# tridivb/attention_based_tbn

Measured on AMD Instinct MI355X. Metric: clips/sec (3-seg RGB+Flow+Audio TBN fwd+bwd), higher is better.
Workload: dtype f32; 1 GPU; BASELINE config 4: RGB+Flow+Audio async, attention off, 3 segments, 224x224 frames + 1.279 s (256x256) spectrogram, train step fwd+loss+bwd+clip+SGD; batch_per_gpu=32, global_batch=32, segments=3, parallelism=single, launch_plans=committed (bench_plans.json)

## Files before the change

### attention_based_tbn_amd/build.py

```python
import os
import subprocess
import sys
from concurrent.futures import ThreadPoolExecutor

HERE = os.path.dirname(os.path.abspath(__file__))
CSRC = os.path.join(HERE, "csrc")
LIB = os.path.join(HERE, "libtbn_hip.so")
SOURCES = ["api.hip", "conv_igemm.hip", "conv_bf16x.hip", "bn.hip", "bn_multi.hip", "bn_res.hip", "pool.hip", "heads.hip", "stft.hip", "engine.hip", "train_ops.hip", "frames.hip", "jpeg.hip", "jpeg_entropy.hip", "audio_load.hip", "inflate.hip", "deflate.hip", "audio_stem.hip", "vgg_ops.hip"]
FLAGS = ["--offload-arch=gfx950", "-O3", "-fPIC", "-std=c++17", "-Wall", "-Wno-unused-function",
         "-mllvm", "-amdgpu-mfma-vgpr-form",
         "-I" + os.path.join(os.path.dirname(HERE), "include")]
if os.environ.get("TBN_DIAG") == "1":
    FLAGS.append("-DTBN_DIAG=1")
if os.environ.get("TBN_EXTRA_FLAGS"):
    FLAGS += os.environ["TBN_EXTRA_FLAGS"].split()
if os.environ.get("TBN_ABLATE") == "1":
    FLAGS.append("-DTBN_ABLATE=1")
if os.environ.get("TBN_EXPERIMENT") == "1":
    FLAGS.append("-DTBN_EXPERIMENT=1")


def _hipcc():
    for c in (os.environ.get("HIPCC"), "/opt/rocm/bin/hipcc", "hipcc"):
        if c and (os.path.isabs(c) and os.path.exists(c) or not os.path.isabs(c)):
            return c
    raise RuntimeError("hipcc not found")


def _stale(target, deps):
    if not os.path.exists(target):
        return True
    t = os.path.getmtime(target)
    return any(os.path.getmtime(d) > t for d in deps)


VARIANT = os.environ.get("TBN_BUILD_VARIANT")
if not VARIANT and any(os.environ.get(k) == "1" for k in ("TBN_EXPERIMENT", "TBN_DIAG", "TBN_ABLATE")):
    VARIANT = "exp" if os.environ.get("TBN_EXPERIMENT") == "1" else ("diag" if os.environ.get("TBN_DIAG") == "1" else "ablate")
OBJDIR = CSRC
if VARIANT:
    _ab = os.path.join(os.path.dirname(HERE), "scripts", "ab")
    OBJDIR = os.path.join(_ab, "obj_" + VARIANT)
    LIB = os.path.join(_ab, "lib_" + VARIANT + ".so")
    os.makedirs(OBJDIR, exist_ok=True)
STAMP = os.path.join(OBJDIR, ".build_flags")


def build(force=False, verbose=True):
    hipcc = _hipcc()
    flagset = " ".join(FLAGS)
    try:
        with open(STAMP) as f:
            if f.read() != flagset:
                force = True
    except OSError:
        force = force or any(os.path.exists(os.path.join(OBJDIR, s.replace(".hip", ".o"))) for s in SOURCES)
    headers = [os.path.join(CSRC, f) for f in os.listdir(CSRC) if f.endswith(".h")]
    headers.append(os.path.join(os.path.dirname(HERE), "include", "tbn_hip.h"))
    objs, jobs = [], []
    for s in SOURCES:
        src = os.path.join(CSRC, s)
        obj = os.path.join(OBJDIR, s.replace(".hip", ".o"))
        objs.append(obj)
        if force or _stale(obj, [src] + headers):
            jobs.append([hipcc] + FLAGS + ["-c", src, "-o", obj])

    def run(cmd):
        if verbose:
            print(" ".join(cmd), flush=True)
        r = subprocess.run(cmd, capture_output=True, text=True)
        if r.returncode != 0:
            raise RuntimeError("hipcc failed:\n" + r.stdout + r.stderr)
        if verbose and r.stderr.strip():
            print(r.stderr, file=sys.stderr)

    with ThreadPoolExecutor(max_workers=min(8, max(1, len(jobs)))) as ex:
        list(ex.map(run, jobs))
    with open(STAMP, "w") as f:
        f.write(flagset)
    if jobs or force or _stale(LIB, objs):
        run([hipcc, "--offload-arch=gfx950", "-shared", "-fPIC", "-o", LIB] + objs)
    return LIB


if __name__ == "__main__":
    print(build(force="--force" in sys.argv))
```

### attention_based_tbn_amd/csrc/bn.hip

```cpp
#include "tbn_common.h"
#include "tbn_kernels.h"
#include "tbn_bn_dev.h"
#include "tbn_pool_dev.h"

static inline int pick_chunk(int P, int rp) {
  int pch = cdiv(P, 512);
  if (pch < 64) pch = 64;
  return cdiv(pch, rp) * rp;
}

__global__ __launch_bounds__(256) void bn_stats_kernel(const float* __restrict__ y, int ld, int P, int C, int pch,
                                                       float* __restrict__ partial) {
  __shared__ float red[2 * 2048];
  const int G = C >> 2, RP = 256 / G;
  const int tid = threadIdx.x, cg = tid % G, rs = tid / G;
  const int p0 = blockIdx.x * pch, p1 = min(P, p0 + pch);
  float4 s1 = make_float4(0, 0, 0, 0), s2 = s1;
  if (rs < RP)
    for (int p = p0 + rs; p < p1; p += RP) {
      const float4 v = *reinterpret_cast<const float4*>(y + (size_t)p * ld + cg * 4);
      s1.x += v.x; s1.y += v.y; s1.z += v.z; s1.w += v.w;
      s2.x = fmaf(v.x, v.x, s2.x); s2.y = fmaf(v.y, v.y, s2.y); s2.z = fmaf(v.z, v.z, s2.z); s2.w = fmaf(v.w, v.w, s2.w);
    }
  if (rs < RP) {
// ... 22 lines not shown
              "bn_stats: P >= 1, C a multiple of 4 in 4..1024, pitch a multiple of 4 and at least C");
  const int rp = 256 / (C / 4), pch = pick_chunk(P, rp), parts = cdiv(P, pch);
  TBN_KLAUNCH(bn_stats_kernel, dim3(parts), dim3(256), 0, st, y, ld, P, C, pch, partial);
  TBN_CHECK_LAUNCH("bn_stats");
  if (nparts) *nparts = parts;
  return TBN_OK;
}

__global__ __launch_bounds__(256) void bn_finalize_kernel(const float* __restrict__ partial, int nparts, int P, int C,
                                                          const float* __restrict__ gamma,
                                                          const float* __restrict__ beta,
                                                          const float* __restrict__ conv_bias, float* running_mean,
                                                          float* running_var, float momentum, float eps,
                                                          float* save_mean, float* save_rstd, float* scale,
                                                          float* shift) {
  __shared__ double red[64 * 32];
  const int tid = threadIdx.x;
  const int c = blockIdx.x * TBN_FIN_CH + tid;
  double s1, s2;
  tbn_sum_partials<TBN_FIN_CH>(partial, C, nparts, blockIdx.x * TBN_FIN_CH, C, red, &s1, &s2);
  if (tid < TBN_FIN_CH && c < C) {
    const double mean = s1 / P;
    double var = s2 / P - mean * mean;
    if (var < 0.0) var = 0.0;
    const float rstd = (float)(1.0 / sqrt(var + (double)eps));
    const float sc = gamma[c] * rstd;
    save_mean[c] = (float)mean;
    save_rstd[c] = rstd;
    scale[c] = sc;
    shift[c] = fmaf(-(float)mean, sc, beta[c]);
    if (running_mean != nullptr) {
      const double unb = P > 1 ? var * ((double)P / (double)(P - 1)) : var;
      const float mean_b = (float)mean + (conv_bias != nullptr ? conv_bias[c] : 0.f);
      running_mean[c] = (1.f - momentum) * running_mean[c] + momentum * mean_b;
      running_var[c] = (1.f - momentum) * running_var[c] + momentum * (float)unb;
    }
  }
}

int tbn_launch_bn_finalize(const float* partial, int nparts, int P, int C, const float* gamma, const float* beta,
                           const float* conv_bias, float* running_mean, float* running_var, float momentum, float eps,
                           float* save_mean, float* save_rstd, float* scale, float* shift, hipStream_t st) {
  TBN_KLAUNCH(bn_finalize_kernel, dim3(cdiv(C, TBN_FIN_CH)), dim3(256), 0, st, partial, nparts, P, C, gamma, beta,
                     conv_bias, running_mean, running_var, momentum, eps, save_mean, save_rstd, scale, shift);
  TBN_CHECK_LAUNCH("bn_finalize");
  return TBN_OK;
}

struct Seg3 {
  Seg s[3];
  int n;
};
struct CSeg3 {
  CSeg s[3];
  int n;
};

__global__ __launch_bounds__(256) void bn_apply_kernel(const float* __restrict__ y, int P, int C,
                                                       const float* __restrict__ scale,
                                                       const float* __restrict__ shift, Seg3 segs, FastDiv divg) {
  const int G = C >> 2;
  const uint32_t total = (uint32_t)P * G;
  for (uint32_t i = blockIdx.x * 256u + threadIdx.x; i < total; i += gridDim.x * 256u) {
    const int p = (int)fdiv(i, divg), c = (int)(i - (uint32_t)p * (uint32_t)G) * 4;
    const float4 v = *reinterpret_cast<const float4*>(y + (size_t)p * C + c);
    const float4 sc = *reinterpret_cast<const float4*>(scale + c);
    const float4 sh = *reinterpret_cast<const float4*>(shift + c);
    float4 z;
// ... 481 lines not shown
```

### attention_based_tbn_amd/csrc/bn_multi.hip

```cpp
#include <cstdlib>
#include <cstring>
#include "tbn_common.h"
#include "tbn_kernels.h"
#include "tbn_bn_dev.h"
#include "tbn_rider_dev.h"

namespace {

__device__ __forceinline__ int find_layer(const int* blk0, int n, int b) {
  int l = 0;
  while (l + 1 < n && b >= blk0[l + 1]) ++l;
  return l;
}

#ifndef TBN_DIAG
#define TBN_DIAG 0
#endif
inline bool diag_skip_fin(int bit) {
#if TBN_DIAG
  static const int mask = getenv("TBN_DIAG_SKIP") ? atoi(getenv("TBN_DIAG_SKIP")) : 0;
  return (mask & bit) != 0;
#else
  (void)bit;
  return false;
#endif
}

inline int ew_grid(size_t items) {
  size_t g = (items + 255) / 256;
  return (int)(g > 4096 ? 4096 : (g < 1 ? 1 : g));
}

}

__global__ __launch_bounds__(256) void bn_finalize_multi_kernel(BnFwdBatch b) {
  __shared__ double red[64 * 32];
  const int li = find_layer(b.fin_blk0, b.n, blockIdx.x);
  const BnFwdLayer& L = b.l[li];
  const int blk = blockIdx.x - b.fin_blk0[li];
  const int C = L.C, P = L.P;
  const int tid = threadIdx.x;
  const int c = blk * TBN_FIN_CH + tid;
  double s1, s2;
  tbn_sum_partials<TBN_FIN_CH>(L.partial, L.pld, L.nparts, blk * TBN_FIN_CH, C, red, &s1, &s2);
  if (tid < TBN_FIN_CH && c < C) {
    const double mean = s1 / P;
    double var = s2 / P - mean * mean;
    if (var < 0.0) var = 0.0;
    const float rstd = (float)(1.0 / sqrt(var + (double)b.eps));
    const float sc = L.gamma[c] * rstd;
    L.save_mean[c] = (float)mean;
    L.save_rstd[c] = rstd;
    L.scale[c] = sc;
    L.shift[c] = fmaf(-(float)mean, sc, L.beta[c]);
    if (L.running_mean != nullptr) {
      const double unb = P > 1 ? var * ((double)P / (double)(P - 1)) : var;
      const float mean_b = (float)mean + (L.conv_bias != nullptr ? L.conv_bias[c] : 0.f);
      L.running_mean[c] = (1.f - b.momentum) * L.running_mean[c] + b.momentum * mean_b;
      L.running_var[c] = (1.f - b.momentum) * L.running_var[c] + b.momentum * (float)unb;
    }
  }
}

__global__ __launch_bounds__(256) void bn_apply_multi_kernel(BnFwdBatch b) {
  const int li = find_layer(b.app_blk0, b.n, blockIdx.x);
  const BnFwdLayer& L = b.l[li];
  const int blk = blockIdx.x - b.app_blk0[li];
  const int p0 = blk * L.app_rows, p1 = min(L.P, p0 + L.app_rows);
  if (L.nseg == 1 && L.seg[0].col_begin == 0) {
    tbn_bn_apply_rows(L.y, L.y_ld, L.seg[0].ptr, L.seg[0].ld, L.scale, L.shift, L.C, p0, p1);
    return;
  }
  const int G = L.C >> 2, RP = 256 / G;
  const int cg = threadIdx.x % G, rs = threadIdx.x / G;
  if (rs >= RP) return;
  const int c = cg * 4;
  const float4 sc = *reinterpret_cast<const float4*>(L.scale + c);
  const float4 sh = *reinterpret_cast<const float4*>(L.shift + c);
  int sg = 0;
  if (L.nseg > 1 && c >= L.seg[1].col_begin) sg = 1;
  if (L.nseg > 2 && c >= L.seg[2].col_begin) sg = 2;
  const float* yp = L.y + (size_t)(p0 + rs) * L.y_ld + c;
  float* zp = L.seg[sg].ptr + (size_t)(p0 + rs) * L.seg[sg].ld + (c - L.seg[sg].col_begin);
  const size_t ystep = (size_t)RP * L.y_ld, zstep = (size_t)RP * L.seg[sg].ld;
  int p = p0 + rs;
  for (; p + 3 * RP < p1; p += 4 * RP) {
    float4 v[4];
#pragma unroll
    for (int k = 0; k < 4; ++k) v[k] = *reinterpret_cast<const float4*>(yp + k * ystep);
#pragma unroll
    for (int k = 0; k < 4; ++k) {
      float4 z;
      z.x = fmaxf(fmaf(v[k].x, sc.x, sh.x), 0.f);
      z.y = fmaxf(fmaf(v[k].y, sc.y, sh.y), 0.f);
      z.z = fmaxf(fmaf(v[k].z, sc.z, sh.z), 0.f);
      z.w = fmaxf(fmaf(v[k].w, sc.w, sh.w), 0.f);
      *reinterpret_cast<float4*>(zp + k * zstep) = z;
    }
    yp += 4 * ystep;
    zp += 4 * zstep;
  }
  for (; p < p1; p += RP) {
    const float4 v = *reinterpret_cast<const float4*>(yp);
    float4 z;
    z.x = fmaxf(fmaf(v.x, sc.x, sh.x), 0.f);
    z.y = fmaxf(fmaf(v.y, sc.y, sh.y), 0.f);
    z.z = fmaxf(fmaf(v.z, sc.z, sh.z), 0.f);
    z.w = fmaxf(fmaf(v.w, sc.w, sh.w), 0.f);
    *reinterpret_cast<float4*>(zp) = z;
    yp += ystep;
    zp += zstep;
  }
}

static inline int apply_rows(int P, int C) {
  const int RP = 256 / (C / 4);
  int it = cdiv(P, RP * 2048);
  if (it < 4) it = 4;
  if (it > 16) it = 16;
  return RP * it;
}

int tbn_launch_bn_fwd_multi(BnFwdBatch& b, hipStream_t st) { return tbn_launch_bn_fwd_multi_defer(b, 0u, nullptr, st); }

int tbn_rider_place(RiderP* r, int gemm_blocks) {
  static const int front = tbn_env_int("TBN_RIDER_FRONT", 0, 0, 1);
  if (r == nullptr || r->nblk <= 0) return gemm_blocks;
  if (front) {
    r->span = (r->nblk + 7) / 8 * 8;
    r->first = 0;
    r->gemm0 = r->span;
  } else {
    r->span = r->nblk;
    r->first = gemm_blocks;
    r->gemm0 = 0;
  }
  return gemm_blocks + r->span;
}

int tbn_launch_bn_fwd_multi_defer(BnFwdBatch& b, unsigned defer_mask, RiderP* rider, hipStream_t st) {
  TBN_REQUIRE(b.n >= 1 && b.n <= TBN_BN_MAXL, "bn_fwd_multi: %d layers", b.n);
  TBN_REQUIRE(defer_mask == 0u || rider != nullptr, "bn_fwd_multi: deferred members need a rider descriptor");
  b.fin_blk0[0] = b.app_blk0[0] = 0;
  for (int i = 0; i < b.n; ++i) {
    BnFwdLayer& L = b.l[i];
    TBN_REQUIRE(L.P >= 1 && L.C >= 4 && L.C % 4 == 0 && L.C <= 1024 && L.y_ld % 4 == 0 && L.y_ld >= L.C && L.pld >= L.C &&
                L.pld % 4 == 0 && L.nparts >= 1 && L.nseg >= 1 && L.nseg <= 3, "bn_fwd_multi: bad P / C / pitch / nparts / nseg");
    for (int s = 0; s < L.nseg; ++s)
      TBN_REQUIRE(L.seg[s].ld % 4 == 0 && L.seg[s].col_begin % 4 == 0, "bn_fwd_multi: segment pitch/offset must be x4");
    b.fin_blk0[i + 1] = b.fin_blk0[i] + cdiv(L.C, TBN_FIN_CH);
    L.app_rows = apply_rows(L.P, L.C);
    b.app_blk0[i + 1] = b.app_blk0[i] + cdiv(L.P, L.app_rows);
  }
  if (!diag_skip_fin(16)) TBN_KLAUNCH(bn_finalize_multi_kernel, dim3(b.fin_blk0[b.n]), dim3(256), 0, st, b);
  TBN_CHECK_LAUNCH("bn_finalize_multi");
  if (defer_mask == 0u) {
    TBN_KLAUNCH(bn_apply_multi_kernel, dim3(b.app_blk0[b.n]), dim3(256), 0, st, b);
    TBN_CHECK_LAUNCH("bn_apply_multi");
    return TBN_OK;
  }
  static thread_local BnFwdBatch now;
  now.n = 0;
  now.momentum = b.momentum;
  now.eps = b.eps;
  now.app_blk0[0] = 0;
  memset(rider, 0, sizeof(*rider));
  rider->kind = 1;
  for (int i = 0; i < b.n; ++i) {
    const BnFwdLayer& L = b.l[i];
    const int blocks = b.app_blk0[i + 1] - b.app_blk0[i];
    if (defer_mask & (1u << i)) {
      TBN_REQUIRE(rider->n < TBN_RIDER_MAXL && L.nseg == 1 && L.seg[0].col_begin == 0, "bn_fwd_multi: rider holds at most %d single-segment layers", TBN_RIDER_MAXL);
      RiderLayer& R = rider->l[rider->n];
      R.y = L.y; R.y_ld = L.y_ld; R.out = L.seg[0].ptr; R.out_ld = L.seg[0].ld;
      R.scale = L.scale; R.shift = L.shift; R.P = L.P; R.C = L.C; R.rows = L.app_rows;
      rider->blk0[rider->n + 1] = rider->blk0[rider->n] + blocks;
      ++rider->n;
    } else {
      now.l[now.n] = L;
      now.app_blk0[now.n + 1] = now.app_blk0[now.n] + blocks;
      ++now.n;
    }
  }
  rider->nblk = rider->blk0[rider->n];
  if (now.n > 0) {
    TBN_KLAUNCH(bn_apply_multi_kernel, dim3(now.app_blk0[now.n]), dim3(256), 0, st, now);
    TBN_CHECK_LAUNCH("bn_apply_multi");
  }
  return TBN_OK;
}

__global__ __launch_bounds__(256) void bn_bwd_reduce_multi_kernel(BnBwdBatch b) {
  __shared__ float red[2 * 2048];
  const int li = find_layer(b.red_blk0, b.n, blockIdx.x);
  const BnBwdLayer& L = b.l[li];
  const int blk = blockIdx.x - b.red_blk0[li];
  const int C = L.C, P = L.P, pch = L.pch;
  const int G = C >> 2, RP = 256 / G;
  const int tid = threadIdx.x, cg = tid % G, rs = tid / G, c = cg * 4;
  const int p0 = blk * pch, p1 = min(P, p0 + pch);
  float4 s1 = make_float4(0, 0, 0, 0), s2 = s1;
  if (rs < RP) {
    int sg = 0;
    if (L.nseg > 1 && c >= L.dz[1].col_begin) sg = 1;
    if (L.nseg > 2 && c >= L.dz[2].col_begin) sg = 2;
    const float* dzp = L.dz[sg].ptr + (c - L.dz[sg].col_begin);
    const int dld = L.dz[sg].ld;
    const float4 sc = *reinterpret_cast<const float4*>(L.scale + c);
// ... 28 lines not shown
    L.partial[((size_t)blk * 2 + 0) * C + cc] = a;
    L.partial[((size_t)blk * 2 + 1) * C + cc] = s;
  }
}

__global__ __launch_bounds__(256) void bn_bwd_finalize_multi_kernel(BnBwdBatch b) {
  __shared__ double red[64 * 32];
  const int li = find_layer(b.fin_blk0, b.n, blockIdx.x);
  const BnBwdLayer& L = b.l[li];
  const int blk = blockIdx.x - b.fin_blk0[li];
  const int C = L.C, P = L.P;
  const int tid = threadIdx.x;
  const int c = blk * TBN_FIN_CH + tid;
  double s1, s2;
  tbn_sum_partials<TBN_FIN_CH>(L.partial, C, L.nparts, blk * TBN_FIN_CH, C, red, &s1, &s2);
  if (tid < TBN_FIN_CH && c < C) {
    const double sc = L.scale[c], rs = L.rstd[c], mu = L.mean[c];
    const double bb = -sc * rs * (s2 / P);
    L.coef[c] = (float)sc;
    L.coef[C + c] = (float)bb;
    L.coef[2 * C + c] = (float)(-sc * (s1 / P) - bb * mu);
    if (L.dgamma) L.dgamma[c] = (float)s2;
    if (L.dbeta) L.dbeta[c] = (float)s1;
    if (L.dbias) L.dbias[c] = 0.f;
  }
}

__global__ __launch_bounds__(256) void bn_bwd_apply_multi_kernel(BnBwdBatch b) {
  const int li = find_layer(b.app_blk0, b.n, blockIdx.x);
  const BnBwdLayer& L = b.l[li];
  const int blk = blockIdx.x - b.app_blk0[li];
  const int p0 = blk * L.app_rows, p1 = min(L.P, p0 + L.app_rows);
  if (L.nseg == 1 && L.dz[0].col_begin == 0) {
    tbn_bn_bwd_apply_rows(L.dz[0].ptr, L.dz[0].ld, L.y, L.y_ld, L.dy, L.scale, L.shift, L.coef, L.C, p0, p1);
    return;
  }
  const int C = L.C, G = C >> 2, RP = 256 / G;
  const int cg = threadIdx.x % G, rs = threadIdx.x / G;
  if (rs >= RP) return;
  const int c = cg * 4;
  int sg = 0;
  if (L.nseg > 1 && c >= L.dz[1].col_begin) sg = 1;
  if (L.nseg > 2 && c >= L.dz[2].col_begin) sg = 2;
  const float4 sc = *reinterpret_cast<const float4*>(L.scale + c);
  const float4 sh = *reinterpret_cast<const float4*>(L.shift + c);
  const float4 ca = *reinterpret_cast<const float4*>(L.coef + c);
  const float4 cb = *reinterpret_cast<const float4*>(L.coef + C + c);
  const float4 cc = *reinterpret_cast<const float4*>(L.coef + 2 * C + c);
  const float* dp = L.dz[sg].ptr + (size_t)(p0 + rs) * L.dz[sg].ld + (c - L.dz[sg].col_begin);
  const float* yp = L.y + (size_t)(p0 + rs) * L.y_ld + c;
  float* op = L.dy + (size_t)(p0 + rs) * L.y_ld + c;
  const size_t dstep = (size_t)RP * L.dz[sg].ld, ystep = (size_t)RP * L.y_ld;
  auto one = [&](const float4 d, const float4 v) {
    float4 o;
    o.x = fmaf(ca.x, fmaf(v.x, sc.x, sh.x) > 0.f ? d.x : 0.f, fmaf(cb.x, v.x, cc.x));
    o.y = fmaf(ca.y, fmaf(v.y, sc.y, sh.y) > 0.f ? d.y : 0.f, fmaf(cb.y, v.y, cc.y));
    o.z = fmaf(ca.z, fmaf(v.z, sc.z, sh.z) > 0.f ? d.z : 0.f, fmaf(cb.z, v.z, cc.z));
    o.w = fmaf(ca.w, fmaf(v.w, sc.w, sh.w) > 0.f ? d.w : 0.f, fmaf(cb.w, v.w, cc.w));
    return o;
  };
  int p = p0 + rs;
  for (; p + 3 * RP < p1; p += 4 * RP) {
    float4 d[4], v[4];
#pragma unroll
    for (int k = 0; k < 4; ++k) {
      d[k] = *reinterpret_cast<const float4*>(dp + k * dstep);
      v[k] = *reinterpret_cast<const float4*>(yp + k * ystep);
// ... 9 lines not shown
    dp += dstep;
    yp += ystep;
    op += ystep;
  }
}

int tbn_launch_bn_bwd_multi(BnBwdBatch& b, hipStream_t st) { return tbn_launch_bn_bwd_multi_defer(b, 0u, nullptr, st); }

int tbn_launch_bn_bwd_multi_defer(BnBwdBatch& b, unsigned defer_mask, RiderP* rider, hipStream_t st) {
  TBN_REQUIRE(b.n >= 1 && b.n <= TBN_BN_MAXL, "bn_bwd_multi: %d layers", b.n);
  TBN_REQUIRE(defer_mask == 0u || rider != nullptr, "bn_bwd_multi: deferred members need a rider descriptor");
  b.red_blk0[0] = b.fin_blk0[0] = b.app_blk0[0] = 0;
  for (int i = 0; i < b.n; ++i) {
    BnBwdLayer& L = b.l[i];
    TBN_REQUIRE(L.P >= 1 && L.C >= 4 && L.C % 4 == 0 && L.C <= 1024 && L.y_ld % 4 == 0 && L.y_ld >= L.C && L.ext_parts >= 0 &&
                L.nseg >= 1 && L.nseg <= 3, "bn_bwd_multi: bad P / C / pitch / ext_parts / nseg");
    for (int s = 0; s < L.nseg; ++s)
      TBN_REQUIRE(L.dz[s].ld % 4 == 0 && L.dz[s].col_begin % 4 == 0, "bn_bwd_multi: segment pitch/offset must be x4");
    {
      const int rp = 256 / (L.C / 4);
      int pch = cdiv(L.P, 512);
      if (pch < 64) pch = 64;
      L.pch = cdiv(pch, rp) * rp;
      L.nparts = cdiv(L.P, L.pch);
    }
    int red_blocks = L.nparts;
    if (L.ext_parts > 0) {
      L.nparts = L.ext_parts;
      red_blocks = 0;
    }
    b.red_blk0[i + 1] = b.red_blk0[i] + red_blocks;
    b.fin_blk0[i + 1] = b.fin_blk0[i] + cdiv(L.C, TBN_FIN_CH);
    L.app_rows = apply_rows(L.P, L.C);
    b.app_blk0[i + 1] = b.app_blk0[i] + cdiv(L.P, L.app_rows);
  }
  if (b.red_blk0[b.n] > 0) {
    TBN_KLAUNCH(bn_bwd_reduce_multi_kernel, dim3(b.red_blk0[b.n]), dim3(256), 0, st, b);
    TBN_CHECK_LAUNCH("bn_bwd_reduce_multi");
  }
  if (!diag_skip_fin(32)) TBN_KLAUNCH(bn_bwd_finalize_multi_kernel, dim3(b.fin_blk0[b.n]), dim3(256), 0, st, b);
  TBN_CHECK_LAUNCH("bn_bwd_finalize_multi");
  if (defer_mask == 0u) {
    TBN_KLAUNCH(bn_bwd_apply_multi_kernel, dim3(b.app_blk0[b.n]), dim3(256), 0, st, b);
    TBN_CHECK_LAUNCH("bn_bwd_apply_multi");
    return TBN_OK;
  }
  static thread_local BnBwdBatch now;
  now.n = 0;
  now.app_blk0[0] = 0;
  memset(rider, 0, sizeof(*rider));
  rider->kind = 2;
  for (int i = 0; i < b.n; ++i) {
    const BnBwdLayer& L = b.l[i];
    const int blocks = b.app_blk0[i + 1] - b.app_blk0[i];
    if (defer_mask & (1u << i)) {
      TBN_REQUIRE(rider->n < TBN_RIDER_MAXL && L.nseg == 1 && L.dz[0].col_begin == 0, "bn_bwd_multi: rider holds at most %d single-segment layers", TBN_RIDER_MAXL);
      RiderLayer& R = rider->l[rider->n];
      R.y = L.y; R.y_ld = L.y_ld; R.out = L.dy; R.out_ld = L.y_ld; R.dz = L.dz[0].ptr; R.dz_ld = L.dz[0].ld;
      R.scale = L.scale; R.shift = L.shift; R.coef = L.coef; R.P = L.P; R.C = L.C; R.rows = L.app_rows;
      rider->blk0[rider->n + 1] = rider->blk0[rider->n] + blocks;
      ++rider->n;
    } else {
      now.l[now.n] = L;
      now.app_blk0[now.n + 1] = now.app_blk0[now.n] + blocks;
      ++now.n;
    }
  }
  rider->nblk = rider->blk0[rider->n];
  if (now.n > 0) {
    TBN_KLAUNCH(bn_bwd_apply_multi_kernel, dim3(now.app_blk0[now.n]), dim3(256), 0, st, now);
    TBN_CHECK_LAUNCH("bn_bwd_apply_multi");
  }
  return TBN_OK;
}
```

### attention_based_tbn_amd/csrc/tbn_bn_dev.h

```cpp
#pragma once
#include "tbn_common.h"

#ifndef TBN_FIN_CH
#define TBN_FIN_CH 16
#endif

template <int CH>
__device__ __forceinline__ void tbn_sum_partials(const float* __restrict__ partial, int pld, int nparts, int c0, int C,
                                                 double* red, double* out_s1, double* out_s2) {
  constexpr int Q = CH / 4, S = 256 / Q, V = Q * 8, G = S / 8;
  static_assert(CH == 4 || CH == 8 || CH == 16, "finalize: 4, 8 or 16 channels per workgroup");
  const int tid = threadIdx.x, cq = tid % Q, slot = tid / Q;
  const int c = c0 + cq * 4;
  double a0 = 0, a1 = 0, a2 = 0, a3 = 0, b0 = 0, b1 = 0, b2 = 0, b3 = 0;
  if (c < C) {
    const float* p = partial + c;
    for (int i = slot; i < nparts; i += 4 * S) {
      float4 u[4], v[4];
#pragma unroll
      for (int k = 0; k < 4; ++k) {
        const int r = i + S * k;
        const bool ok = r < nparts;
        const size_t rr = (size_t)(ok ? r : i);
        u[k] = *reinterpret_cast<const float4*>(p + (rr * 2 + 0) * pld);
        v[k] = *reinterpret_cast<const float4*>(p + (rr * 2 + 1) * pld);
        if (!ok) u[k] = v[k] = make_float4(0.f, 0.f, 0.f, 0.f);
      }
#pragma unroll
      for (int k = 0; k < 4; ++k) {
        a0 += (double)u[k].x; a1 += (double)u[k].y; a2 += (double)u[k].z; a3 += (double)u[k].w;
        b0 += (double)v[k].x; b1 += (double)v[k].y; b2 += (double)v[k].z; b3 += (double)v[k].w;
      }
    }
  }
  double* r = red + slot * V + cq * 8;
  r[0] = a0; r[1] = a1; r[2] = a2; r[3] = a3;
  r[4] = b0; r[5] = b1; r[6] = b2; r[7] = b3;
  __syncthreads();
// ... 19 lines not shown
```

### attention_based_tbn_amd/csrc/tbn_kernels.h

```cpp
#pragma once
#include "tbn_common.h"
#include <hip/hip_ext.h>
#include <type_traits>

enum { CONV_EPI_PLAIN = 0, CONV_EPI_STATS = 1, CONV_EPI_EVAL = 2 };
enum {
  CONV_FLAG_ACCUM = 1,
  CONV_FLAG_RELU = 2,
  CONV_FLAG_HALO = 4,
  CONV_FLAG_DMA = 8,
  CONV_FLAG_SK4 = 16,
  CONV_FLAG_BF16X6 = 32,
  CONV_FLAG_BF16X3 = 64,
  CONV_FLAG_BF16X_PLANES = 128,
  CONV_FLAG_DESC_OUT2 = 256
};

#define TBN_CONV_MAXSEG 4
struct RedSeg {
  const float* y;
  float* partial;
  const float* stats;
  int y_ld, col_begin, C, c_off;
  unsigned y_bytes;
// ... 14 lines not shown
  int nred;
  int red_chan;
  int red_row0;
  int N, H, W;
  int OH, OW;
  int Cin;
  int Cout;
  int R, S, stride, pad, up;
  int M, K;
  int cp;
  int tiles_m, tiles_n;
  int mode, flags;
  double alg_flops;
  int stages;
  int halo;
  unsigned in_bytes, wt_bytes;
  unsigned seg_bytes[TBN_CONV_MAXSEG];
  int OHs, OWs;
  int out_sy, out_oy, out_sx, out_ox;
  int in_sy, in_sx;
  int Krow;
  int ntaps;
  int tap_dy[9], tap_dx[9];
  int tap_koff[9];
  int tap_off[9];
  int ty0, tny, tx0, tnx;
  FastDiv div_ohw, div_ow;
  FastDiv div_rl4;
  const float* fold_scale;
  const float* fold_shift;
};

#define TBN_RIDER_MAXL 3
struct RiderLayer {
  const float* y;
  const float* dz;
  float* out;
  const float* scale;
  const float* shift;
  const float* coef;
  int y_ld, dz_ld, out_ld, P, C, rows;
};
struct RiderP {
  int span;
  int first;
  int gemm0;
  int nblk;
  int kind;
  int n;
  int blk0[TBN_RIDER_MAXL + 1];
  RiderLayer l[TBN_RIDER_MAXL];
};
int tbn_rider_place(RiderP* r, int gemm_blocks);

struct WgradP {
  const float* dy;
  const float* x;
  float* out;
  int dy_ld, x_ld;
  int N, H, W, OH, OW;
  int Cin, Cout;
  int R, S, stride, pad;
  int taps;
  int M, K;
  int cp, rl;
  int tiles_co, tiles_ci;
  int rows_per_split;
  int mt, nt;
  FastDiv div_ohw, div_ow, div_rl4;
  unsigned mul_ow;
  unsigned r64;
  unsigned frame_bytes;
  unsigned fb_lo, fb_hi;
  unsigned row_step, col_step;
// ... 137 lines not shown
};
int tbn_launch_weight_flip_transpose_all(const float* w, float* wt, const FlipTab& tab, hipStream_t st);

int tbn_launch_bn_stats(const float* y, int ld, int P, int C, float* partial, int* nparts, hipStream_t st);
int tbn_bn_stats_parts(int P, int C);
int tbn_launch_bn_finalize(const float* partial, int nparts, int P, int C, const float* gamma, const float* beta,
                           const float* conv_bias, float* running_mean, float* running_var, float momentum, float eps,
                           float* save_mean, float* save_rstd, float* scale, float* shift, hipStream_t st);
int tbn_launch_bn_apply(const float* y, int P, int C, const float* scale, const float* shift, const Seg* segs,
                        int nseg, hipStream_t st);
int tbn_launch_bn_apply_maxpool(const float* y, int N, int H, int W, int C, const float* scale, const float* shift,
                                float* out, int out_ld, unsigned char* argmax, int OH, int OW, int stride, int pad,
                                hipStream_t st);
int tbn_launch_bn_bwd_reduce_pooled(const float* dpooled, int dpooled_ld, const unsigned char* argmax, int N, int H,
                                    int W, int OH, int OW, int stride, int pad, const float* y, int C,
                                    const float* scale, const float* shift, const float* mean, const float* rstd,
                                    float* partial, hipStream_t st);
int tbn_bn_bwd_pooled_parts(int N, int H, int W, int C, int stride, int pad);
int tbn_launch_bn_bwd_apply_pooled(const float* dpooled, int dpooled_ld, const unsigned char* argmax, int N, int H, int W,
                                   int OH, int OW, int stride, int pad, const float* y, int C, const float* scale,
                                   const float* shift, const float* coef, float* dy, hipStream_t st);
#define TBN_BN_MAXL 4
struct BnFwdLayer {
  const float* y;
  int y_ld;
  int P, C;
  const float* partial;
  int pld, nparts;
  const float *gamma, *beta, *conv_bias;
  float *running_mean, *running_var, *save_mean, *save_rstd, *scale, *shift;
  Seg seg[3];
  int nseg;
  int app_rows;
};
struct BnFwdBatch {
  int n;
  float momentum, eps;
  BnFwdLayer l[TBN_BN_MAXL];
  int fin_blk0[TBN_BN_MAXL + 1], app_blk0[TBN_BN_MAXL + 1];
};
struct BnBwdLayer {
  CSeg dz[3];
  int nseg;
  const float* y;
  float* dy;
  int y_ld;
  int P, C;
  const float *scale, *shift, *mean, *rstd;
  float* partial;
  int ext_parts;
  float* coef;
  float *dgamma, *dbeta, *dbias;
  int pch, nparts;
  int app_rows;
};
struct BnBwdBatch {
  int n;
  BnBwdLayer l[TBN_BN_MAXL];
  int red_blk0[TBN_BN_MAXL + 1], fin_blk0[TBN_BN_MAXL + 1], app_blk0[TBN_BN_MAXL + 1];
};
int tbn_launch_bn_fwd_multi(BnFwdBatch& b, hipStream_t st);
int tbn_launch_bn_bwd_multi(BnBwdBatch& b, hipStream_t st);
int tbn_launch_bn_fwd_multi_defer(BnFwdBatch& b, unsigned defer_mask, RiderP* rider, hipStream_t st);
int tbn_launch_bn_bwd_multi_defer(BnBwdBatch& b, unsigned defer_mask, RiderP* rider, hipStream_t st);
bool tbn_prof_enabled();
int tbn_launch_bn_fold(const float* gamma, const float* beta, const float* mean, const float* var, const float* bias,
                       float eps, float* scale, float* shift, int C, hipStream_t st);
int tbn_bn_bwd_parts(int P, int C);
int tbn_launch_bn_bwd_reduce(const CSeg* dz, int nseg, const float* y, int P, int C, const float* scale,
                             const float* shift, const float* mean, const float* rstd, float* partial, hipStream_t st);
int tbn_launch_bn_bwd_finalize(const float* partial, int nparts, int P, int C, const float* scale, const float* mean,
                               const float* rstd, float* coef, float* dgamma, float* dbeta, float* dbias,
                               hipStream_t st);
int tbn_launch_bn_bwd_apply(const CSeg* dz, int nseg, const float* y, int P, int C, const float* scale,
                            const float* shift, const float* coef, float* dy, hipStream_t st);

int tbn_launch_maxpool_fwd(const float* in, int in_ld, float* out, int out_ld, uint8_t* argmax, int N, int H, int W,
                           int C, int OH, int OW, int stride, int pad, hipStream_t st);
int tbn_launch_maxpool_bwd(const float* dout, int dout_ld, const uint8_t* argmax, float* din, int din_ld, int N,
                           int H, int W, int C, int OH, int OW, int stride, int pad, int accumulate, hipStream_t st);
int tbn_launch_avgpool3_fwd(const float* in, int in_ld, float* out, int out_ld, int N, int H, int W, int C,
                            int accumulate, hipStream_t st);
int tbn_launch_spatial_mean_fwd(const float* in, int in_ld, float* out, int out_ld, int N, int H, int W, int C,
                                int freq_only, hipStream_t st);
int tbn_launch_spatial_mean_bwd(const float* dout, int dout_ld, float* din, int din_ld, int N, int H, int W, int C,
                                int freq_only, hipStream_t st);
int tbn_launch_nchw_to_s2d_pad(const float* in, float* out, int N, int C, int H, int W, hipStream_t st);
// ... 6 lines not shown
```

### attention_based_tbn_amd/csrc/tbn_rider_dev.h

```cpp
#pragma once
#include "tbn_common.h"
#include "tbn_kernels.h"

__device__ __forceinline__ void tbn_bn_apply_rows(const float* __restrict__ y, int y_ld, float* __restrict__ z, int z_ld,
                                                  const float* __restrict__ scale, const float* __restrict__ shift, int C,
                                                  int p0, int p1) {
  const int G = C >> 2, RP = 256 / G;
  const int cg = threadIdx.x % G, rs = threadIdx.x / G;
  if (rs >= RP) return;
  const int c = cg * 4;
  const float4 sc = *reinterpret_cast<const float4*>(scale + c);
  const float4 sh = *reinterpret_cast<const float4*>(shift + c);
  const float* yp = y + (size_t)(p0 + rs) * y_ld + c;
  float* zp = z + (size_t)(p0 + rs) * z_ld + c;
  const size_t ystep = (size_t)RP * y_ld, zstep = (size_t)RP * z_ld;
  int p = p0 + rs;
  for (; p + 3 * RP < p1; p += 4 * RP) {
    float4 v[4];
#pragma unroll
    for (int k = 0; k < 4; ++k) v[k] = tbn_ld4<(TBN_BN_NT & 1) != 0>(yp + k * ystep);
#pragma unroll
    for (int k = 0; k < 4; ++k) {
      float4 o;
      o.x = fmaxf(fmaf(v[k].x, sc.x, sh.x), 0.f);
      o.y = fmaxf(fmaf(v[k].y, sc.y, sh.y), 0.f);
      o.z = fmaxf(fmaf(v[k].z, sc.z, sh.z), 0.f);
      o.w = fmaxf(fmaf(v[k].w, sc.w, sh.w), 0.f);
      tbn_st4<(TBN_BN_NT & 4) != 0>(zp + k * zstep, o);
    }
    yp += 4 * ystep;
    zp += 4 * zstep;
  }
  for (; p < p1; p += RP) {
    const float4 v = tbn_ld4<(TBN_BN_NT & 1) != 0>(yp);
    float4 o;
    o.x = fmaxf(fmaf(v.x, sc.x, sh.x), 0.f);
    o.y = fmaxf(fmaf(v.y, sc.y, sh.y), 0.f);
    o.z = fmaxf(fmaf(v.z, sc.z, sh.z), 0.f);
    o.w = fmaxf(fmaf(v.w, sc.w, sh.w), 0.f);
    tbn_st4<(TBN_BN_NT & 4) != 0>(zp, o);
    yp += ystep;
    zp += zstep;
  }
}

__device__ __forceinline__ void tbn_bn_bwd_apply_rows(const float* __restrict__ dz, int dz_ld, const float* y, int y_ld,
                                                      float* dy, const float* __restrict__ scale,
                                                      const float* __restrict__ shift, const float* __restrict__ coef, int C,
                                                      int p0, int p1) {
  const int G = C >> 2, RP = 256 / G;
  const int cg = threadIdx.x % G, rs = threadIdx.x / G;
  if (rs >= RP) return;
  const int c = cg * 4;
  const float4 sc = *reinterpret_cast<const float4*>(scale + c);
  const float4 sh = *reinterpret_cast<const float4*>(shift + c);
  const float4 ca = *reinterpret_cast<const float4*>(coef + c);
  const float4 cb = *reinterpret_cast<const float4*>(coef + C + c);
  const float4 cc = *reinterpret_cast<const float4*>(coef + 2 * C + c);
  const float* dp = dz + (size_t)(p0 + rs) * dz_ld + c;
  const float* yp = y + (size_t)(p0 + rs) * y_ld + c;
  float* op = dy + (size_t)(p0 + rs) * y_ld + c;
  const size_t dstep = (size_t)RP * dz_ld, ystep = (size_t)RP * y_ld;
  auto one = [&](const float4 d, const float4 v) {
    float4 o;
    o.x = fmaf(ca.x, fmaf(v.x, sc.x, sh.x) > 0.f ? d.x : 0.f, fmaf(cb.x, v.x, cc.x));
    o.y = fmaf(ca.y, fmaf(v.y, sc.y, sh.y) > 0.f ? d.y : 0.f, fmaf(cb.y, v.y, cc.y));
    o.z = fmaf(ca.z, fmaf(v.z, sc.z, sh.z) > 0.f ? d.z : 0.f, fmaf(cb.z, v.z, cc.z));
    o.w = fmaf(ca.w, fmaf(v.w, sc.w, sh.w) > 0.f ? d.w : 0.f, fmaf(cb.w, v.w, cc.w));
    return o;
  };
  int p = p0 + rs;
  for (; p + 3 * RP < p1; p += 4 * RP) {
    float4 d[4], v[4];
#pragma unroll
    for (int k = 0; k < 4; ++k) {
      d[k] = tbn_ld4<(TBN_BN_NT & 2) != 0>(dp + k * dstep);
      v[k] = tbn_ld4<(TBN_BN_NT & 2) != 0>(yp + k * ystep);
    }
#pragma unroll
    for (int k = 0; k < 4; ++k) tbn_st4<(TBN_BN_NT & 4) != 0>(op + k * ystep, one(d[k], v[k]));
    dp += 4 * dstep;
    yp += 4 * ystep;
    op += 4 * ystep;
  }
  for (; p < p1; p += RP) {
    tbn_st4<(TBN_BN_NT & 4) != 0>(op, one(tbn_ld4<(TBN_BN_NT & 2) != 0>(dp), tbn_ld4<(TBN_BN_NT & 2) != 0>(yp)));
    dp += dstep;
    yp += ystep;
    op += ystep;
  }
}

__device__ __forceinline__ void tbn_rider_block(const RiderP& r, int rb) {
  int li = 0;
  while (li + 1 < r.n && rb >= r.blk0[li + 1]) ++li;
  const RiderLayer& L = r.l[li];
  const int blk = rb - r.blk0[li];
  const int p0 = blk * L.rows, p1 = min(L.P, p0 + L.rows);
  if (r.kind == 1)
    tbn_bn_apply_rows(L.y, L.y_ld, L.out, L.out_ld, L.scale, L.shift, L.C, p0, p1);
  else
    tbn_bn_bwd_apply_rows(L.dz, L.dz_ld, L.y, L.y_ld, L.out, L.scale, L.shift, L.coef, L.C, p0, p1);
}

#define TBN_RIDER_DISPATCH(r, bid)                                   \
  const int rider_rb__ = (int)blockIdx.x - (r).first;               \
  if (rider_rb__ >= 0 && rider_rb__ < (r).span) {                   \
    if (rider_rb__ < (r).nblk) tbn_rider_block((r), rider_rb__);    \
    return;                                                          \
  }                                                                  \
  const int bid = (int)blockIdx.x - (r).gemm0;
```

Before: 909.9 clips/s.

## Use buffer loads/stores and precomputed row map in BN apply kernels

Rewrites the BN forward and backward apply row loops to use raw buffer-resource loads and stores with 32-bit offsets, and replaces the per-thread divide/modulo lane mapping with a host-precomputed multiply-shift. It also disables SLP vectorization for the BN and pool sources, forces scalar v_fma_f32 through inline asm in the backward apply, and makes the running-stat blend non-contracted. The aim is to cut 64-bit address arithmetic, integer-division overhead and the scheduling problems caused by packed math. The cost is that tensors whose block span exceeds 2GB are now rejected, and the tail loop now takes a per-row bounds branch.

```diff
diff --git a/attention_based_tbn_amd/build.py b/attention_based_tbn_amd/build.py
--- a/attention_based_tbn_amd/build.py
+++ b/attention_based_tbn_amd/build.py
@@ -10,6 +10,10 @@
 FLAGS = ["--offload-arch=gfx950", "-O3", "-fPIC", "-std=c++17", "-Wall", "-Wno-unused-function",
          "-mllvm", "-amdgpu-mfma-vgpr-form",
          "-I" + os.path.join(os.path.dirname(HERE), "include")]
+NO_SLP_SOURCES = ("bn.hip", "bn_multi.hip", "pool.hip")
+ALLOW_SLP = os.environ.get("TBN_ALLOW_SLP") == "1"
+if ALLOW_SLP:
+    FLAGS.append("-DTBN_F32_SINGLE=0")
 if os.environ.get("TBN_DIAG") == "1":
     FLAGS.append("-DTBN_DIAG=1")
 if os.environ.get("TBN_EXTRA_FLAGS"):
@@ -63,7 +67,8 @@
         obj = os.path.join(OBJDIR, s.replace(".hip", ".o"))
         objs.append(obj)
         if force or _stale(obj, [src] + headers):
-            jobs.append([hipcc] + FLAGS + ["-c", src, "-o", obj])
+            extra = ["-fno-slp-vectorize"] if s in NO_SLP_SOURCES and not ALLOW_SLP else []
+            jobs.append([hipcc] + FLAGS + extra + ["-c", src, "-o", obj])
 
     def run(cmd):
         if verbose:
diff --git a/attention_based_tbn_amd/csrc/bn.hip b/attention_based_tbn_amd/csrc/bn.hip
--- a/attention_based_tbn_amd/csrc/bn.hip
+++ b/attention_based_tbn_amd/csrc/bn.hip
@@ -78,8 +78,8 @@
     if (running_mean != nullptr) {
       const double unb = P > 1 ? var * ((double)P / (double)(P - 1)) : var;
       const float mean_b = (float)mean + (conv_bias != nullptr ? conv_bias[c] : 0.f);
-      running_mean[c] = (1.f - momentum) * running_mean[c] + momentum * mean_b;
-      running_var[c] = (1.f - momentum) * running_var[c] + momentum * (float)unb;
+      running_mean[c] = tbn_blend(momentum, running_mean[c], mean_b);
+      running_var[c] = tbn_blend(momentum, running_var[c], (float)unb);
     }
   }
 }
diff --git a/attention_based_tbn_amd/csrc/bn_multi.hip b/attention_based_tbn_amd/csrc/bn_multi.hip
--- a/attention_based_tbn_amd/csrc/bn_multi.hip
+++ b/attention_based_tbn_amd/csrc/bn_multi.hip
@@ -56,8 +56,8 @@
     if (L.running_mean != nullptr) {
       const double unb = P > 1 ? var * ((double)P / (double)(P - 1)) : var;
       const float mean_b = (float)mean + (L.conv_bias != nullptr ? L.conv_bias[c] : 0.f);
-      L.running_mean[c] = (1.f - b.momentum) * L.running_mean[c] + b.momentum * mean_b;
-      L.running_var[c] = (1.f - b.momentum) * L.running_var[c] + b.momentum * (float)unb;
+      L.running_mean[c] = tbn_blend(b.momentum, L.running_mean[c], mean_b);
+      L.running_var[c] = tbn_blend(b.momentum, L.running_var[c], (float)unb);
     }
   }
 }
@@ -68,7 +68,7 @@
   const int blk = blockIdx.x - b.app_blk0[li];
   const int p0 = blk * L.app_rows, p1 = min(L.P, p0 + L.app_rows);
   if (L.nseg == 1 && L.seg[0].col_begin == 0) {
-    tbn_bn_apply_rows(L.y, L.y_ld, L.seg[0].ptr, L.seg[0].ld, L.scale, L.shift, L.C, p0, p1);
+    tbn_bn_apply_rows(L.y, L.y_ld, L.seg[0].ptr, L.seg[0].ld, L.scale, L.shift, L.C, L.map, p0, p1);
     return;
   }
   const int G = L.C >> 2, RP = 256 / G;
@@ -121,6 +121,8 @@
   return RP * it;
 }
 
+static inline bool apply_block_fits(int rows, int ld) { return (size_t)rows * (size_t)ld * 4u < (1ull << 31); }
+
 int tbn_launch_bn_fwd_multi(BnFwdBatch& b, hipStream_t st) { return tbn_launch_bn_fwd_multi_defer(b, 0u, nullptr, st); }
 
 int tbn_rider_place(RiderP* r, int gemm_blocks) {
@@ -150,6 +152,9 @@
       TBN_REQUIRE(L.seg[s].ld % 4 == 0 && L.seg[s].col_begin % 4 == 0, "bn_fwd_multi: segment pitch/offset must be x4");
     b.fin_blk0[i + 1] = b.fin_blk0[i] + cdiv(L.C, TBN_FIN_CH);
     L.app_rows = apply_rows(L.P, L.C);
+    L.map = tbn_make_rowmap(L.C);
+    for (int s = 0; s < L.nseg; ++s)
+      TBN_REQUIRE(apply_block_fits(L.app_rows, L.y_ld) && apply_block_fits(L.app_rows, L.seg[s].ld), "bn_fwd_multi: pitch too wide");
     b.app_blk0[i + 1] = b.app_blk0[i] + cdiv(L.P, L.app_rows);
   }
   if (!diag_skip_fin(16)) TBN_KLAUNCH(bn_finalize_multi_kernel, dim3(b.fin_blk0[b.n]), dim3(256), 0, st, b);
@@ -173,7 +178,7 @@
       TBN_REQUIRE(rider->n < TBN_RIDER_MAXL && L.nseg == 1 && L.seg[0].col_begin == 0, "bn_fwd_multi: rider holds at most %d single-segment layers", TBN_RIDER_MAXL);
       RiderLayer& R = rider->l[rider->n];
       R.y = L.y; R.y_ld = L.y_ld; R.out = L.seg[0].ptr; R.out_ld = L.seg[0].ld;
-      R.scale = L.scale; R.shift = L.shift; R.P = L.P; R.C = L.C; R.rows = L.app_rows;
+      R.scale = L.scale; R.shift = L.shift; R.P = L.P; R.C = L.C; R.rows = L.app_rows; R.map = L.map;
       rider->blk0[rider->n + 1] = rider->blk0[rider->n] + blocks;
       ++rider->n;
     } else {
@@ -268,7 +273,7 @@
   const int blk = blockIdx.x - b.app_blk0[li];
   const int p0 = blk * L.app_rows, p1 = min(L.P, p0 + L.app_rows);
   if (L.nseg == 1 && L.dz[0].col_begin == 0) {
-    tbn_bn_bwd_apply_rows(L.dz[0].ptr, L.dz[0].ld, L.y, L.y_ld, L.dy, L.scale, L.shift, L.coef, L.C, p0, p1);
+    tbn_bn_bwd_apply_rows(L.dz[0].ptr, L.dz[0].ld, L.y, L.y_ld, L.dy, L.scale, L.shift, L.coef, L.C, L.map, p0, p1);
     return;
   }
   const int C = L.C, G = C >> 2, RP = 256 / G;
@@ -344,6 +349,9 @@
     b.red_blk0[i + 1] = b.red_blk0[i] + red_blocks;
     b.fin_blk0[i + 1] = b.fin_blk0[i] + cdiv(L.C, TBN_FIN_CH);
     L.app_rows = apply_rows(L.P, L.C);
+    L.map = tbn_make_rowmap(L.C);
+    for (int s = 0; s < L.nseg; ++s)
+      TBN_REQUIRE(apply_block_fits(L.app_rows, L.y_ld) && apply_block_fits(L.app_rows, L.dz[s].ld), "bn_bwd_multi: pitch too wide");
     b.app_blk0[i + 1] = b.app_blk0[i] + cdiv(L.P, L.app_rows);
   }
   if (b.red_blk0[b.n] > 0) {
@@ -369,7 +377,7 @@
       TBN_REQUIRE(rider->n < TBN_RIDER_MAXL && L.nseg == 1 && L.dz[0].col_begin == 0, "bn_bwd_multi: rider holds at most %d single-segment layers", TBN_RIDER_MAXL);
       RiderLayer& R = rider->l[rider->n];
       R.y = L.y; R.y_ld = L.y_ld; R.out = L.dy; R.out_ld = L.y_ld; R.dz = L.dz[0].ptr; R.dz_ld = L.dz[0].ld;
-      R.scale = L.scale; R.shift = L.shift; R.coef = L.coef; R.P = L.P; R.C = L.C; R.rows = L.app_rows;
+      R.scale = L.scale; R.shift = L.shift; R.coef = L.coef; R.P = L.P; R.C = L.C; R.rows = L.app_rows; R.map = L.map;
       rider->blk0[rider->n + 1] = rider->blk0[rider->n] + blocks;
       ++rider->n;
     } else {
diff --git a/attention_based_tbn_amd/csrc/tbn_bn_dev.h b/attention_based_tbn_amd/csrc/tbn_bn_dev.h
--- a/attention_based_tbn_amd/csrc/tbn_bn_dev.h
+++ b/attention_based_tbn_amd/csrc/tbn_bn_dev.h
@@ -4,6 +4,12 @@
 #ifndef TBN_FIN_CH
 #define TBN_FIN_CH 16
 #endif
+
+__device__ __forceinline__ float tbn_blend(float m, float old, float now) {
+#pragma clang fp contract(off)
+  const float a = (1.f - m) * old, b = m * now;
+  return a + b;
+}
 
 template <int CH>
 __device__ __forceinline__ void tbn_sum_partials(const float* __restrict__ partial, int pld, int nparts, int c0, int C,
diff --git a/attention_based_tbn_amd/csrc/tbn_kernels.h b/attention_based_tbn_amd/csrc/tbn_kernels.h
--- a/attention_based_tbn_amd/csrc/tbn_kernels.h
+++ b/attention_based_tbn_amd/csrc/tbn_kernels.h
@@ -70,6 +70,15 @@
 };
 
 #define TBN_RIDER_MAXL 3
+struct TbnRowMap {
+  int gmul, rp;
+};
+static inline TbnRowMap tbn_make_rowmap(int C) {
+  TbnRowMap m;
+  m.gmul = 65536 / (C / 4) + 1;
+  m.rp = 256 / (C / 4);
+  return m;
+}
 struct RiderLayer {
   const float* y;
   const float* dz;
@@ -78,6 +87,7 @@
   const float* shift;
   const float* coef;
   int y_ld, dz_ld, out_ld, P, C, rows;
+  TbnRowMap map;
 };
 struct RiderP {
   int span;
@@ -281,6 +291,7 @@
   Seg seg[3];
   int nseg;
   int app_rows;
+  TbnRowMap map;
 };
 struct BnFwdBatch {
   int n;
@@ -302,6 +313,7 @@
   float *dgamma, *dbeta, *dbias;
   int pch, nparts;
   int app_rows;
+  TbnRowMap map;
 };
 struct BnBwdBatch {
   int n;
diff --git a/attention_based_tbn_amd/csrc/tbn_rider_dev.h b/attention_based_tbn_amd/csrc/tbn_rider_dev.h
--- a/attention_based_tbn_amd/csrc/tbn_rider_dev.h
+++ b/attention_based_tbn_amd/csrc/tbn_rider_dev.h
@@ -1,24 +1,60 @@
 #pragma once
 #include "tbn_common.h"
 #include "tbn_kernels.h"
+#include "tbn_conv_dev.h"
+
+__device__ void tbn_llvm_buffer_store_f32x4(f32x4 data, i32x4 srsrc, int voffset, int soffset, int aux) __asm(
+    "llvm.amdgcn.raw.buffer.store.v4f32");
+template <bool NT>
+__device__ __forceinline__ float4 tbn_buf_ld4(i32x4 r, unsigned voff, unsigned soff) {
+  const f32x4 v = tbn_llvm_buffer_load_f32x4(r, (int)voff, (int)soff, NT ? 2 : 0);
+  return make_float4(v.x, v.y, v.z, v.w);
+}
+template <bool NT>
+__device__ __forceinline__ void tbn_buf_st4(i32x4 r, unsigned voff, unsigned soff, const float4 o) {
+  const f32x4 v = {o.x, o.y, o.z, o.w};
+  tbn_llvm_buffer_store_f32x4(v, r, (int)voff, (int)soff, NT ? 2 : 0);
+}
+
+#ifndef TBN_F32_SINGLE
+#define TBN_F32_SINGLE 1
+#endif
+__device__ __forceinline__ float tbn_fma1(float a, float b, float c) {
+#if TBN_F32_SINGLE
+  float r;
+  asm("v_fma_f32 %0, %1, %2, %3" : "=v"(r) : "v"(a), "v"(b), "v"(c));
+  return r;
+#else
+  return fmaf(a, b, c);
+#endif
+}
+
+__device__ __forceinline__ bool tbn_row_lane(const TbnRowMap m, int G, int& rs, int& cg) {
+  rs = (int)(((unsigned)threadIdx.x * (unsigned)m.gmul) >> 16);
+  cg = (int)threadIdx.x - rs * G;
+  return rs < m.rp;
+}
 
 __device__ __forceinline__ void tbn_bn_apply_rows(const float* __restrict__ y, int y_ld, float* __restrict__ z, int z_ld,
                                                   const float* __restrict__ scale, const float* __restrict__ shift, int C,
-                                                  int p0, int p1) {
-  const int G = C >> 2, RP = 256 / G;
-  const int cg = threadIdx.x % G, rs = threadIdx.x / G;
-  if (rs >= RP) return;
-  const int c = cg * 4;
-  const float4 sc = *reinterpret_cast<const float4*>(scale + c);
-  const float4 sh = *reinterpret_cast<const float4*>(shift + c);
-  const float* yp = y + (size_t)(p0 + rs) * y_ld + c;
-  float* zp = z + (size_t)(p0 + rs) * z_ld + c;
-  const size_t ystep = (size_t)RP * y_ld, zstep = (size_t)RP * z_ld;
-  int p = p0 + rs;
-  for (; p + 3 * RP < p1; p += 4 * RP) {
+                                                  const TbnRowMap m, int p0, int p1) {
+  constexpr bool LNT = (TBN_BN_NT & 1) != 0, SNT = (TBN_BN_NT & 4) != 0;
+  const int G = C >> 2, RP = m.rp, nrow = p1 - p0;
+  int rs, cg;
+  if (!tbn_row_lane(m, G, rs, cg)) return;
+  const i32x4 cr_sc = make_rsrc(scale, (unsigned)C * 4u), cr_sh = make_rsrc(shift, (unsigned)C * 4u);
+  const float4 sc = tbn_buf_ld4<false>(cr_sc, (unsigned)cg * 16u, 0u);
+  const float4 sh = tbn_buf_ld4<false>(cr_sh, (unsigned)cg * 16u, 0u);
+  const i32x4 yr = make_rsrc(y + (size_t)p0 * y_ld, ((unsigned)(nrow - 1) * (unsigned)y_ld + (unsigned)C) * 4u);
+  const i32x4 zr = make_rsrc(z + (size_t)p0 * z_ld, ((unsigned)(nrow - 1) * (unsigned)z_ld + (unsigned)C) * 4u);
+  const unsigned yv = (unsigned)(rs * y_ld + cg * 4) * 4u, zv = (unsigned)(rs * z_ld + cg * 4) * 4u;
+  const unsigned ystep = (unsigned)(RP * y_ld) * 4u, zstep = (unsigned)(RP * z_ld) * 4u;
+  unsigned ys = 0u, zs = 0u;
+  int b = 0;
+  for (; b + 4 * RP <= nrow; b += 4 * RP) {
     float4 v[4];
 #pragma unroll
-    for (int k = 0; k < 4; ++k) v[k] = tbn_ld4<(TBN_BN_NT & 1) != 0>(yp + k * ystep);
+    for (int k = 0; k < 4; ++k) v[k] = tbn_buf_ld4<LNT>(yr, yv, ys + k * ystep);
 #pragma unroll
     for (int k = 0; k < 4; ++k) {
       float4 o;
@@ -26,68 +62,72 @@
       o.y = fmaxf(fmaf(v[k].y, sc.y, sh.y), 0.f);
       o.z = fmaxf(fmaf(v[k].z, sc.z, sh.z), 0.f);
       o.w = fmaxf(fmaf(v[k].w, sc.w, sh.w), 0.f);
-      tbn_st4<(TBN_BN_NT & 4) != 0>(zp + k * zstep, o);
+      tbn_buf_st4<SNT>(zr, zv, zs + k * zstep, o);
     }
-    yp += 4 * ystep;
-    zp += 4 * zstep;
+    ys += 4u * ystep;
+    zs += 4u * zstep;
   }
-  for (; p < p1; p += RP) {
-    const float4 v = tbn_ld4<(TBN_BN_NT & 1) != 0>(yp);
-    float4 o;
-    o.x = fmaxf(fmaf(v.x, sc.x, sh.x), 0.f);
-    o.y = fmaxf(fmaf(v.y, sc.y, sh.y), 0.f);
-    o.z = fmaxf(fmaf(v.z, sc.z, sh.z), 0.f);
-    o.w = fmaxf(fmaf(v.w, sc.w, sh.w), 0.f);
-    tbn_st4<(TBN_BN_NT & 4) != 0>(zp, o);
-    yp += ystep;
-    zp += zstep;
+  for (; b < nrow; b += RP) {
+    if (b + rs < nrow) {
+      const float4 v = tbn_buf_ld4<LNT>(yr, yv, ys);
+      float4 o;
+      o.x = fmaxf(fmaf(v.x, sc.x, sh.x), 0.f);
+      o.y = fmaxf(fmaf(v.y, sc.y, sh.y), 0.f);
+      o.z = fmaxf(fmaf(v.z, sc.z, sh.z), 0.f);
+      o.w = fmaxf(fmaf(v.w, sc.w, sh.w), 0.f);
+      tbn_buf_st4<SNT>(zr, zv, zs, o);
+    }
+    ys += ystep;
+    zs += zstep;
   }
 }
 
 __device__ __forceinline__ void tbn_bn_bwd_apply_rows(const float* __restrict__ dz, int dz_ld, const float* y, int y_ld,
                                                       float* dy, const float* __restrict__ scale,
                                                       const float* __restrict__ shift, const float* __restrict__ coef, int C,
-                                                      int p0, int p1) {
-  const int G = C >> 2, RP = 256 / G;
-  const int cg = threadIdx.x % G, rs = threadIdx.x / G;
-  if (rs >= RP) return;
-  const int c = cg * 4;
-  const float4 sc = *reinterpret_cast<const float4*>(scale + c);
-  const float4 sh = *reinterpret_cast<const float4*>(shift + c);
-  const float4 ca = *reinterpret_cast<const float4*>(coef + c);
-  const float4 cb = *reinterpret_cast<const float4*>(coef + C + c);
-  const float4 cc = *reinterpret_cast<const float4*>(coef + 2 * C + c);
-  const float* dp = dz + (size_t)(p0 + rs) * dz_ld + c;
-  const float* yp = y + (size_t)(p0 + rs) * y_ld + c;
-  float* op = dy + (size_t)(p0 + rs) * y_ld + c;
-  const size_t dstep = (size_t)RP * dz_ld, ystep = (size_t)RP * y_ld;
+                                                      const TbnRowMap m, int p0, int p1) {
+  constexpr bool LNT = (TBN_BN_NT & 2) != 0, SNT = (TBN_BN_NT & 4) != 0;
+  const int G = C >> 2, RP = m.rp, nrow = p1 - p0;
+  int rs, cg;
+  if (!tbn_row_lane(m, G, rs, cg)) return;
+  const i32x4 cr_sc = make_rsrc(scale, (unsigned)C * 4u), cr_sh = make_rsrc(shift, (unsigned)C * 4u);
+  const i32x4 cr_co = make_rsrc(coef, (unsigned)C * 12u);
+  const float4 sc = tbn_buf_ld4<false>(cr_sc, (unsigned)cg * 16u, 0u);
+  const float4 sh = tbn_buf_ld4<false>(cr_sh, (unsigned)cg * 16u, 0u);
+  const float4 ca = tbn_buf_ld4<false>(cr_co, (unsigned)cg * 16u, 0u);
+  const float4 cb = tbn_buf_ld4<false>(cr_co, (unsigned)cg * 16u, (unsigned)C * 4u);
+  const float4 cc = tbn_buf_ld4<false>(cr_co, (unsigned)cg * 16u, (unsigned)C * 8u);
+  const i32x4 dr = make_rsrc(dz + (size_t)p0 * dz_ld, ((unsigned)(nrow - 1) * (unsigned)dz_ld + (unsigned)C) * 4u);
+  const i32x4 yr = make_rsrc(y + (size_t)p0 * y_ld, ((unsigned)(nrow - 1) * (unsigned)y_ld + (unsigned)C) * 4u);
+  const i32x4 orr = make_rsrc(dy + (size_t)p0 * y_ld, ((unsigned)(nrow - 1) * (unsigned)y_ld + (unsigned)C) * 4u);
+  const unsigned dv = (unsigned)(rs * dz_ld + cg * 4) * 4u, yv = (unsigned)(rs * y_ld + cg * 4) * 4u;
+  const unsigned dstep = (unsigned)(RP * dz_ld) * 4u, ystep = (unsigned)(RP * y_ld) * 4u;
   auto one = [&](const float4 d, const float4 v) {
     float4 o;
-    o.x = fmaf(ca.x, fmaf(v.x, sc.x, sh.x) > 0.f ? d.x : 0.f, fmaf(cb.x, v.x, cc.x));
-    o.y = fmaf(ca.y, fmaf(v.y, sc.y, sh.y) > 0.f ? d.y : 0.f, fmaf(cb.y, v.y, cc.y));
-    o.z = fmaf(ca.z, fmaf(v.z, sc.z, sh.z) > 0.f ? d.z : 0.f, fmaf(cb.z, v.z, cc.z));
-    o.w = fmaf(ca.w, fmaf(v.w, sc.w, sh.w) > 0.f ? d.w : 0.f, fmaf(cb.w, v.w, cc.w));
+    o.x = tbn_fma1(ca.x, tbn_fma1(v.x, sc.x, sh.x) > 0.f ? d.x : 0.f, tbn_fma1(cb.x, v.x, cc.x));
+    o.y = tbn_fma1(ca.y, tbn_fma1(v.y, sc.y, sh.y) > 0.f ? d.y : 0.f, tbn_fma1(cb.y, v.y, cc.y));
+    o.z = tbn_fma1(ca.z, tbn_fma1(v.z, sc.z, sh.z) > 0.f ? d.z : 0.f, tbn_fma1(cb.z, v.z, cc.z));
+    o.w = tbn_fma1(ca.w, tbn_fma1(v.w, sc.w, sh.w) > 0.f ? d.w : 0.f, tbn_fma1(cb.w, v.w, cc.w));
     return o;
   };
-  int p = p0 + rs;
-  for (; p + 3 * RP < p1; p += 4 * RP) {
+  unsigned ds = 0u, ys = 0u;
+  int b = 0;
+  for (; b + 4 * RP <= nrow; b += 4 * RP) {
     float4 d[4], v[4];
 #pragma unroll
     for (int k = 0; k < 4; ++k) {
-      d[k] = tbn_ld4<(TBN_BN_NT & 2) != 0>(dp + k * dstep);
-      v[k] = tbn_ld4<(TBN_BN_NT & 2) != 0>(yp + k * ystep);
+      d[k] = tbn_buf_ld4<LNT>(dr, dv, ds + k * dstep);
+      v[k] = tbn_buf_ld4<LNT>(yr, yv, ys + k * ystep);
     }
 #pragma unroll
-    for (int k = 0; k < 4; ++k) tbn_st4<(TBN_BN_NT & 4) != 0>(op + k * ystep, one(d[k], v[k]));
-    dp += 4 * dstep;
-    yp += 4 * ystep;
-    op += 4 * ystep;
+    for (int k = 0; k < 4; ++k) tbn_buf_st4<SNT>(orr, yv, ys + k * ystep, one(d[k], v[k]));
+    ds += 4u * dstep;
+    ys += 4u * ystep;
   }
-  for (; p < p1; p += RP) {
-    tbn_st4<(TBN_BN_NT & 4) != 0>(op, one(tbn_ld4<(TBN_BN_NT & 2) != 0>(dp), tbn_ld4<(TBN_BN_NT & 2) != 0>(yp)));
-    dp += dstep;
-    yp += ystep;
-    op += ystep;
+  for (; b < nrow; b += RP) {
+    if (b + rs < nrow) tbn_buf_st4<SNT>(orr, yv, ys, one(tbn_buf_ld4<LNT>(dr, dv, ds), tbn_buf_ld4<LNT>(yr, yv, ys)));
+    ds += dstep;
+    ys += ystep;
   }
 }
 
@@ -98,9 +138,9 @@
   const int blk = rb - r.blk0[li];
   const int p0 = blk * L.rows, p1 = min(L.P, p0 + L.rows);
   if (r.kind == 1)
-    tbn_bn_apply_rows(L.y, L.y_ld, L.out, L.out_ld, L.scale, L.shift, L.C, p0, p1);
+    tbn_bn_apply_rows(L.y, L.y_ld, L.out, L.out_ld, L.scale, L.shift, L.C, L.map, p0, p1);
   else
-    tbn_bn_bwd_apply_rows(L.dz, L.dz_ld, L.y, L.y_ld, L.out, L.scale, L.shift, L.coef, L.C, p0, p1);
+    tbn_bn_bwd_apply_rows(L.dz, L.dz_ld, L.y, L.y_ld, L.out, L.scale, L.shift, L.coef, L.C, L.map, p0, p1);
 }
 
 #define TBN_RIDER_DISPATCH(r, bid)                                   \
```

New measurement: 915.8 clips/s, median of 6. No clear change (+0.6%).
